# AlexanderGSC/gmres

Measured on AMD Instinct MI355X. Metric: Arnoldi iters/sec + HBM GB/s, 4096² Poisson-2D fp64, GMRES(m=95), higher is better.
Workload: dtype f64

## Files before the change

### gmres_amd/_native.py

```python
from __future__ import annotations

import ctypes
import os
import sys
import re

PKG = os.path.dirname(os.path.abspath(__file__))
LIB_DIR = os.environ.get("GK_LIB_DIR") or os.path.join(PKG, "lib")
HIP_SO = os.path.join(LIB_DIR, "libgmres_hip.so")
FHOST_SO = os.path.join(LIB_DIR, "libgmres_fhost.so")
HEADER = os.path.join(os.path.dirname(PKG), "include", "gmres_hip.h")

GK_OK = 0
GK_ERR_COMM = -6
GK_TUNE_PROJ_NT = 0
GK_TUNE_STENCIL_BLOCKS = 2
GK_TUNE_SR_BLOCKS = 28
GK_TUNE_SR_TWO_LEVEL = 29
GK_TUNE_XCHG_TIMEOUT_MS = 7
GK_TUNE_RES, GK_TUNE_RES_R2, GK_TUNE_RES_SHARE, GK_TUNE_RES_TIMEOUT_MS = 8, 9, 10, 11
GK_TUNE_VERR_ORDER = 14
GK_TUNE_HH_FUSE = 15
GK_TUNE_CHEB_STEN = 16
GK_TUNE_SPIN_WAIT = 18
GK_TUNE_GRAPH = 19
GK_TUNE_RES_QDEF = 20
GK_TUNE_RES_PC = 21
GK_TUNE_RES_FOLD = 22
GK_TUNE_RES_BLOCK = 23
GK_TUNE_WATCHDOG_MS = 24
GK_TUNE_HH_NORM_ORDER = 25
GK_TUNE_RES_PF = 27
GK_PREC_IDENTITY, GK_PREC_CBPR2, GK_PREC_CHEB = 0, 1, 2
(GK_KID_PROJ, GK_KID_STENCIL, GK_KID_SCALE, GK_KID_UPDATE, GK_KID_COMM, GK_KID_OTHER, GK_KID_RES, GK_KID_PREC,
 GK_KID_HALO, GK_KID_GRAPH) = range(10)
GK_KID_SR = 10
SR_PASS_NAMES = ["sr_cg_p", "sr_cg_x", "sr_cg_z", "sr_bi_p", "sr_bi_pc", "sr_bi_s", "sr_bi_sc", "sr_st1", "sr_st2",
                 "sr_bi_x", "sr_bi_pe", "sr_bi_se", "sr_dot", "sr_cg_xz", "sr_bi_pz", "sr_bi_sz"]
KID_NAMES = ["proj", "stencil", "scale", "update", "comm", "other", "res", "prec", "halo", "graph"] + SR_PASS_NAMES
GK_SR_PCG, GK_SR_BICGSTAB = 0, 1
COMM_KINDS = {0: None, 1: "rccl", 2: "local-group", 3: "xgmi-device-exchange"}
RES_VARIANTS = {0: None, 1: "prefetch", 2: "pairs", 3: "pairs+lds", 4: "w-only", 5: "w+column", 6: "blocked"}
RES_INFO_KEYS = ["variant", "G", "r2", "l2", "pf", "cw", "wo", "nt", "r2e", "l2e", "lds", "nres2", "unused12", "cheb_sten", "wt", "blk"]

c_int, c_double, c_ll, c_vp = ctypes.c_int, ctypes.c_double, ctypes.c_longlong, ctypes.c_void_p
_dp = ctypes.POINTER(ctypes.c_double)
_ip = ctypes.POINTER(ctypes.c_int)

_hip = None
_fhost = None


class GkError(RuntimeError):
    pass


def header_symbols() -> list[str]:
    txt = open(HEADER).read()
    return sorted(set(re.findall(r"^\s*(?:int|const char \*)\s*(gk_\w+)\s*\(", txt, re.M)))


_SIGS = {
    "gk_last_error": (ctypes.c_char_p, []),
    "gk_version": (c_int, []),
    "gk_runtime_info": (c_int, [_ip, _ip, _ip, ctypes.c_char_p, ctypes.c_char_p, c_int]),
    "gk_create": (c_int, [c_int, c_int, c_int, c_int, c_int, ctypes.POINTER(c_vp)]),
    "gk_destroy": (c_int, [c_vp]),
    "gk_comm_unique_id": (c_int, [ctypes.c_char_p]),
    "gk_comm_init": (c_int, [c_vp, c_int, c_int, c_int, ctypes.c_char_p]),
    "gk_local_size": (c_int, [c_vp, ctypes.POINTER(c_ll)]),
    "gk_comm_info": (c_int, [c_vp, _ip, _ip]),
    "gk_peer_info": (c_int, [c_int, c_int, _ip, _ip, _ip]),
    "gk_comm_latency": (c_int, [c_vp, c_int, _dp, _dp]),
    "gk_group_create": (c_int, [c_int, ctypes.POINTER(c_vp)]),
    "gk_group_destroy": (c_int, [c_vp]),
    "gk_comm_init_local": (c_int, [c_vp, c_vp, c_int, c_int]),
    "gk_comm_init_xgmi": (c_int, [c_vp, c_int, c_int, c_int]),
    "gk_xchg_handle": (c_int, [c_vp, ctypes.c_char_p]),
    "gk_xchg_open": (c_int, [c_vp, ctypes.c_char_p]),
    "gk_xchg_local": (c_int, [c_vp]),
    "gk_xchg_enable": (c_int, [c_vp, c_int]),
    "gk_xchg_selftest": (c_int, [c_vp, c_int]),
    "gk_set_precond": (c_int, [c_vp, c_int, _dp, c_int, c_int]),
    "gk_set_rhs": (c_int, [c_vp, _dp]),
    "gk_set_rhs_ones": (c_int, [c_vp]),
    "gk_rhs_norm": (c_int, [c_vp, _dp]),
    "gk_zero_x": (c_int, [c_vp]),
    "gk_get_x": (c_int, [c_vp, _dp]),
    "gk_get_basis": (c_int, [c_vp, c_int, c_int, _dp]),
    "gk_set_x": (c_int, [c_vp, _dp]),
    "gk_apply": (c_int, [c_vp, c_int, _dp, _dp]),
    "gk_true_residual": (c_int, [c_vp, _dp]),
    "gk_mgs_cycle_start": (c_int, [c_vp, _dp]),
    "gk_mgs_step": (c_int, [c_vp, c_int, _dp]),
    "gk_mgs_step_async": (c_int, [c_vp, c_int]),
    "gk_mgs_step_wait": (c_int, [c_vp, c_int, _dp]),
# ... 157 lines not shown
```

### gmres_amd/csrc/gk_api.hip

```cpp
#include <dlfcn.h>
#include <hip/hip_runtime.h>
#include <rccl/rccl.h>

#include <algorithm>
#include <atomic>
#include <chrono>
#include <cmath>
#include <condition_variable>
#include <cstdarg>
#include <cstdlib>
#include <mutex>
#include <cstdio>
#include <cstring>
#include <deque>
#include <string>
#include <vector>

#include "../../include/gmres_hip.h"
#include "gk_blk.hpp"
#include "gk_kernels.hpp"
#include "gk_sr.hpp"

using gk::i64;

// ... 54 lines not shown
    hipStream_t st = nullptr;
    double *V = nullptr;
    double *w = nullptr, *z = nullptr, *aux = nullptr, *dA = nullptr, *dB = nullptr;
    double *x = nullptr, *b = nullptr, *vj = nullptr, *hlo = nullptr, *hhi = nullptr;
    double *dh = nullptr;
    double *zline = nullptr;
    double *red = nullptr;
    double *hcol = nullptr;
    double *ydev = nullptr;
    double *hb = nullptr;
    double *scal = nullptr;
    double *hcol_host = nullptr;
    double *hall = nullptr;
    double *hallh = nullptr;
    double *hallh_dev = nullptr;
    std::vector<hipEvent_t> ev_step;
    double *Vb = nullptr;
    double *gram_slab = nullptr, *gram_out = nullptr;
    short2 *gram_pairs = nullptr;
    int gram_nblk = 0;
    int pkind = GK_PREC_IDENTITY, pdeg = 8;
    double p0 = 8.2, p1 = 0.2;
    int nranks = 1, rank = 0, max_lines = 0;
    int min_lines = 0;
    ncclComm_t comm = nullptr;
    bool comm_ok = false;
    gk_group *lg = nullptr;
    hipEvent_t lev_a = nullptr, lev_b = nullptr;
    double *lscratch = nullptr;
    gk::u64 *xs_buf = nullptr;
    i64 xs_words = 0;
    gk::XsPeers xs_peers{};
    std::vector<void *> xs_mapped;
    bool xs_ready = false, xs_on = false, xs_broken = false;
    unsigned xs_seq = 0, xs_hseq = 0;
    int *xs_err = nullptr, *xs_err_dev = nullptr;
    long long xs_tick_per_ms = 100000;
    int xs_timeout_ms = 20000;
    gk::u64 xs_timeout = 0;
    gk::u64 *res_gath = nullptr;
    double *res_gm = nullptr;
    int tune_res_blk = 1;
    int tune_res_pf = 0;
    int pend_res_blk = 0, pend_res_pf = -1;
    int watchdog_ms = 0;
    bool broken = false;
    unsigned *hold_word = nullptr, *hold_word_dev = nullptr;
    int *res_err = nullptr, *res_err_dev = nullptr;
    unsigned res_tag = 1;
    int res_cus = 0;
    int tune_res = -1;
    int tune_res_r2 = 0;
    int tune_res_lds = 1;
    int tune_res_wonly = -1;
    int tune_verr_order = 1;
    int tune_hh_fuse = 1;
    int tune_hh_norm_order = 0;
    int res_share = 1;
    int res_timeout_ms = 20000;
    bool res_broken = false;
    gk::u64 *res_stamps = nullptr;
    bool res_split = false;
    gk::u64 *res_trace = nullptr;
    int res_trace_j = 0, res_trace_mode = -1;
    int res_trace_g = 0, res_trace_np = 0;
    int vec = 2, JT = 16;
    dim3 sgrid;
    int sr_JT = 64, tune_sr_blocks = 0;
    int tune_sr_two = 1;
    bool sr_two = false;
    dim3 sr_sgrid;
    int np_sr = 0;
    int np_st = 0, np_pj = 0, nblk_stream = 0;
    int last_np = 0;
    int tune_cheb_fused = 1;
    int tune_cheb_sten = 1;
    int tune_spin_wait = 1;
    int tune_graph = 1;
    int tune_res_qdef = -1;
    int tune_res_pc = -1;
    int tune_res_fold = 1;
    std::vector<hipGraphExec_t> gstep;
    std::vector<unsigned> gxs;
    int gkey = -1;
    unsigned graph_seq0 = 0;
    unsigned *xs_seqdev = nullptr;
    bool capturing = false;
    int tune_nt = -1, tune_pj_blocks = 0, tune_st_blocks = 0;
    bool nt_auto = false;
    int tune_blocked = 0, tune_unr = 0;
    int prof_every = 1;
    bool prof_on_step = true;
    bool cycle_mgs = false, cycle_hh = false;
    double beta0 = -1.0;
    bool prof = false;
    std::vector<hipEvent_t> ev0, ev1;
    std::vector<int> evk;
    int nev = 0;
    double prof_ms[GK_NKID] = {0};
    long long prof_n[GK_NKID] = {0};
    gk::SrDev *sr_dev = nullptr;
    gk::SrMirror *sr_mir = nullptr, *sr_mir_dev = nullptr;
    double *sr_hist = nullptr;
    int sr_hist_len = 0;
    int sr_solver = -1, sr_par = 0, sr_queued = 0, sr_maxit = 0;
    std::deque<hipEvent_t> sr_pend;
// ... 440 lines not shown
    else
        launch_proj_u<NT, 4>(c, mode, w, va, vb, pin, npin, pout, hslot, coef, tail0, hstore);
}

int proj(gk_ctx *c, int mode, double *w, const double *va, const double *vb, const double *pin,
         int npin, double *pout, double *hslot, double coef, i64 tail0 = 0, int hstore = 0) {
    ProfScope ps(c, GK_KID_PROJ);
    if (c->tune_nt > 0 || (c->tune_nt < 0 && c->nt_auto))
        launch_proj<true>(c, mode, w, va, vb, pin, npin, pout, hslot, coef, tail0, hstore);
    else
        launch_proj<false>(c, mode, w, va, vb, pin, npin, pout, hslot, coef, tail0, hstore);
    LAUNCHCHK();
    return GK_OK;
}

int scale(gk_ctx *c, double *out, const double *w, const double *pin, int npin, double *hslot,
          double *hcopy = nullptr, const double *hsrc = nullptr, int ncopy = 0, bool pin_norm = false) {
    ProfScope ps(c, GK_KID_SCALE);
    gk::k_scale<<<c->nblk_stream, gk::TPB, 0, c->st>>>(out, w, pin, npin, hslot, c->nloc, hcopy, hsrc, ncopy,
                                                       pin_norm ? 1 : 0);
    LAUNCHCHK();
    return GK_OK;
}

int norm2_seq(gk_ctx *c, const double *x, i64 n, double *out) {
    ProfScope ps(c, GK_KID_OTHER);
    gk::k_norm2_seq<<<1, gk::TPB, 0, c->st>>>(x, n, out);
    LAUNCHCHK();
    return GK_OK;
}

int finalize(gk_ctx *c, const double *pin, int npin, double *out, int take_sqrt) {
    ProfScope ps(c, GK_KID_OTHER);
    gk::k_finalize<<<1, gk::TPB, 0, c->st>>>(pin, npin, out, take_sqrt);
    LAUNCHCHK();
    return GK_OK;
}

constexpr int RES_LDS_MIN = 96 * 1024;
constexpr int RES_L2 = 18;
constexpr int RES_R2_BIG = 12;

#ifndef GK_RES_RW
#define GK_RES_RW 89
#endif
#ifndef GK_RES_LW
#define GK_RES_LW 39
#endif
constexpr int RES_RW = GK_RES_RW, RES_LW = GK_RES_LW, RES_LW_HH = 38;
#ifndef GK_RES_RW_HH
#define GK_RES_RW_HH 90
#endif
constexpr int RES_RW_HH = GK_RES_RW_HH;

struct ResPlan {
    int G = 0, r2 = 0, l2 = 0;
    int r2e = 0, l2e = 0;
    bool pf = false, nt = false, cw = false, wo = false;
    bool pc = false;
    bool pcs = false;
    int blk = 0;
    int bvar = -1;
    int wt = 0;
    i64 nres2 = 0;
    int lds = 0;
};

#ifndef GK_RES_PC_NT
#define GK_RES_PC_NT 512
#endif
#ifndef GK_RES_PC_WB
#define GK_RES_PC_WB (GK_RES_PC_NT == 512 ? 4 : 8)
#endif
#ifndef GK_RES_PC_WB_HH
#define GK_RES_PC_WB_HH (GK_RES_PC_NT == 512 ? 4 : 6)
#endif
#ifndef GK_RES_PC_TOUCH
#define GK_RES_PC_TOUCH 0
#endif
#ifndef GK_RES_PC_RX
#define GK_RES_PC_RX (GK_RES_PC_NT == 512 ? 4 : 26)
#endif
constexpr int RES_PC_NT = GK_RES_PC_NT;
static_assert(RES_PC_NT == 256 || RES_PC_NT == 512, "column-cache workgroups of one or two waves per SIMD");
#ifndef GK_RES_PC_RX_MGS
#define GK_RES_PC_RX_MGS (GK_RES_PC_NT == 512 ? 6 : GK_RES_PC_RX)
#endif
constexpr int RES_PC_RW = RES_PC_NT == 512 ? 32 : 64, RES_PC_RX = GK_RES_PC_RX, RES_PC_LX = RES_PC_NT == 512 ? 19 : 38;
constexpr int RES_PC_RX_MGS = GK_RES_PC_RX_MGS;
constexpr int RES_PC_WB = GK_RES_PC_WB, RES_PC_WB_HH = GK_RES_PC_WB_HH, RES_PC_TOUCH = GK_RES_PC_TOUCH;
#ifndef GK_RES_PC_SMALL
#define GK_RES_PC_SMALL 1
#endif
constexpr bool RES_PCS = GK_RES_PC_SMALL != 0 && RES_PC_NT == 512;
constexpr int RES_PCS_RW = 16, RES_PCS_RX = 16, RES_PCS_LX = 0;

i64 pc_bytes(i64 n2, int G, bool hh) {
    if (RES_PCS && n2 <= (i64)G * RES_PCS_RW * RES_PC_NT) return 8 * n2;
    const int rx = hh ? RES_PC_RX : RES_PC_RX_MGS;
    const i64 cap = (i64)G * RES_PC_RW * RES_PC_NT, cached = (i64)G * (rx + RES_PC_LX) * RES_PC_NT;
    const i64 r = std::min(n2, cap), c = std::min(r, cached);
    return 8 * c + 16 * (r - c) + 32 * (n2 - r);
}

i64 pairs_bytes(i64 n2, int G) {
    const i64 rp = (i64)G * RES_R2_BIG * gk::RT, lp = (i64)G * RES_L2 * gk::RT;
    auto clamp = [](i64 v) { return v < 0 ? (i64)0 : v; };
    const i64 pr = std::min(n2, rp), pl = std::min(clamp(n2 - rp), lp), ps = clamp(n2 - rp - lp);
    return 8 * pr + 16 * pl + 32 * ps;
}

i64 wonly_bytes(i64 n2, int G) {
    const i64 rw = (i64)G * (RES_RW + RES_LW) * gk::WT;
    const i64 wr = std::min(n2, rw), ws = n2 > rw ? n2 - rw : 0;
    return 16 * wr + 32 * ws;
}

bool wonly_pays(i64 n2, int G) { return wonly_bytes(n2, G) < pairs_bytes(n2, G); }

void plan_resident(i64 nloc, int gmax, int cap, int tune_lds, int tune_wonly, bool hh, bool nt, ResPlan &p,
                   int tune_pc = -1, int tune_blk = 1, int tune_pf = 0) {
    const i64 n2 = nloc / 2;
    const i64 dcw = gk::RT - 64;
    const int gcw = (int)std::max<i64>(1, std::min<i64>(gmax, (n2 + 2 * dcw - 1) / (2 * dcw)));
    const i64 need = (n2 + (i64)gcw * dcw - 1) / ((i64)gcw * dcw);
    p = ResPlan{};
    static const int pfs[] = {2, 4, 8};
    for (int s : pfs)
        if (s <= cap && (p.r2 == 0 || p.r2 < need)) p.r2 = s;
    auto spread = [&](i64 dt, int rmax, int lmax) {
        const i64 nchf = n2 / dt, G = p.G;
        p.r2e = (int)std::min<i64>(rmax, (nchf + G - 1) / G);
        const i64 rest = std::max<i64>(0, nchf - G * p.r2e);
        p.l2e = (int)std::min<i64>(lmax, (rest + G - 1) / G);
        p.nres2 = std::min<i64>(nchf, G * (p.r2e + p.l2e)) * dt;
    };
    const int var = gk::blk_variant((n2 + (i64)gmax * 512 - 1) / ((i64)gmax * 512));
    const bool pf = !hh && tune_blk == 1 && var != gk::BLK_WONLY && tune_pf > 0;
    if (!hh && (tune_blk > 1 || pf)) {
        p.G = gmax;
        const gk::BlkGeom g = gk::blk_geom(var, tune_blk);
        p.blk = tune_blk;
        p.bvar = var;
        p.wt = g.nt;
        spread(g.nt, g.rw, g.lw);
        p.r2 = g.rx;
        p.l2 = g.lx;
        p.lds = (g.lw + tune_blk * (g.lx + g.pfx)) * g.nt * (int)sizeof(double2);
        p.nt = true;
        return;
    }
    const bool pc_fits = n2 <= (i64)gmax * RES_PC_RW * RES_PC_NT;
    const i64 other_bytes = std::min(pairs_bytes(n2, gmax), wonly_bytes(n2, gmax));
    const bool pc_pays = pc_fits && (RES_PC_NT == 512 ? pc_bytes(n2, gmax, hh) < other_bytes
                                                      : 3 * pc_bytes(n2, gmax, hh) <= 2 * other_bytes);
    if (p.r2 >= need || cap < RES_R2_BIG) {
        p.G = gcw;
        p.pf = p.cw = true;
        spread(dcw, p.r2, 0);
    } else if (tune_wonly <= 0 && (tune_pc > 0 ? pc_fits : (tune_pc < 0 && pc_pays))) {
        p.G = gmax;
        p.pc = true;
        p.wt = RES_PC_NT;
        spread(RES_PC_NT, RES_PC_RW, 0);
        p.pcs = RES_PCS && p.r2e <= RES_PCS_RW;
        p.r2 = p.pcs ? RES_PCS_RX : (hh ? RES_PC_RX : RES_PC_RX_MGS);
        p.l2 = p.pcs ? RES_PCS_LX : RES_PC_LX;
        p.lds = p.l2 * RES_PC_NT * (int)sizeof(double2);
        p.nt = true;
        return;
    } else if (tune_wonly > 0 || (tune_wonly < 0 && wonly_pays(n2, gmax))) {
        p.G = gmax;
        p.wo = true;
        p.wt = gk::WT;
        p.r2 = 0;
        spread(gk::WT, hh ? RES_RW_HH : RES_RW, hh ? RES_LW_HH : RES_LW);
        p.lds = (hh ? RES_LW_HH : RES_LW) * gk::WT * (int)sizeof(double2);
        p.nt = true;
        return;
    } else {
        p.G = gmax;
        p.r2 = RES_R2_BIG;
        const i64 dt = gk::RT, regs = (i64)p.G * RES_R2_BIG * dt;
        p.l2 = (tune_lds && n2 / dt * dt > regs) ? RES_L2 : 0;
        spread(dt, RES_R2_BIG, p.l2);
    }
    p.lds = std::max<int>(RES_LDS_MIN, p.l2 * (p.cw ? gk::RT - 64 : gk::RT) * (int)sizeof(double2));
    p.wt = gk::RT;
    p.nt = nt;
}

bool nt_auto_for(i64 max_nloc) { return max_nloc * 8 > (i64)48 * 1024 * 1024; }

bool res_plan(gk_ctx *c, ResPlan &p, bool hh = false) {
    if (c->tune_res == 0 || c->res_broken || c->m > gk::RHMAX || c->res_cus <= 0 || c->res_gath == nullptr)
        return false;
    if (collective(c) && !(c->xs_on && c->nranks > 1)) return false;
    if (c->tune_res < 0 && c->res_share > 1) return false;
    const int gmax = std::max(1, std::min(gk::RGMAX, c->res_cus / std::max(1, c->res_share)));
    const int cap = c->tune_res_r2 > 0 ? c->tune_res_r2 : RES_R2_BIG;
    plan_resident(c->nloc, gmax, cap, c->tune_res_lds, c->tune_res_wonly, hh,
                  c->tune_nt > 0 || (c->tune_nt < 0 && c->nt_auto), p, c->tune_res_pc, c->tune_res_blk, c->tune_res_pf);
    if (p.wo && !hh && c->m + 1 > gk::WO_HMAX) return false;
    return true;
}

enum { RPI_VARIANT = 0, RPI_G, RPI_R2, RPI_L2, RPI_PF, RPI_CW, RPI_WO, RPI_NT, RPI_R2E, RPI_L2E, RPI_LDS, RPI_NRES2, RPI_UNUSED12,
       RPI_CHEB_STEN, RPI_WT, RPI_BLK };
void plan_info(const ResPlan &p, bool on, long long *info) {
    for (int k = 0; k < GK_RES_INFO_LEN; ++k) info[k] = 0;
    if (!on) return;
    info[RPI_VARIANT] = p.bvar >= 0 ? GK_RES_BLOCKED
                        : p.pc    ? GK_RES_WCOL
                                  : (p.wo ? GK_RES_WONLY
                                          : (p.pf ? GK_RES_PREFETCH : (p.l2 > 0 ? GK_RES_PAIRS_LDS : GK_RES_PAIRS)));
    info[RPI_BLK] = p.bvar >= 0 ? p.blk : 1;
    info[RPI_G] = p.G;
    info[RPI_R2] = p.r2;
    info[RPI_L2] = p.l2;
    info[RPI_PF] = p.pf;
    info[RPI_CW] = p.cw;
    info[RPI_WO] = p.wo;
    info[RPI_NT] = p.nt;
    info[RPI_R2E] = p.r2e;
    info[RPI_L2E] = p.l2e;
    info[RPI_LDS] = p.lds;
    info[RPI_NRES2] = p.nres2;
    info[RPI_WT] = p.wt;
}

constexpr int ATTR_DEVS = 64;

template <int R2, int L2, bool PF, bool NT, bool CW, int MODE>
int launch_res_m(gk_ctx *c, const ResPlan &p, const gk::ResArgs &a) {
    static std::atomic<int> attr[ATTR_DEVS];
    if (c->dev < 0 || c->dev >= ATTR_DEVS) return set_err(GK_ERR_ARG, "device id %d out of range", c->dev);
    if (attr[c->dev].load() < p.lds) {
        HIPCHK(hipFuncSetAttribute(reinterpret_cast<const void *>(&gk::k_mgs_res<R2, L2, PF, NT, CW, MODE>),
                                   hipFuncAttributeMaxDynamicSharedMemorySize, p.lds));
        attr[c->dev] = p.lds;
    }
    gk::k_mgs_res<R2, L2, PF, NT, CW, MODE><<<p.G, gk::RT, p.lds, c->st>>>(a);
    LAUNCHCHK();
    return GK_OK;
}

template <int R2, int L2, bool PF, bool NT, bool CW>
int launch_res_t(gk_ctx *c, const ResPlan &p, const gk::ResArgs &a) {
    switch (a.mode) {
        case gk::RES_HH_UP: return launch_res_m<R2, L2, PF, NT, CW, gk::RES_HH_UP>(c, p, a);
        case gk::RES_HH_DOWN: return launch_res_m<R2, L2, PF, NT, CW, gk::RES_HH_DOWN>(c, p, a);
        default: return launch_res_m<R2, L2, PF, NT, CW, gk::RES_MGS>(c, p, a);
    }
}

template <int MODE>
int launch_wres_m(gk_ctx *c, const ResPlan &p, const gk::ResArgs &a) {
    constexpr int RW = MODE == gk::RES_MGS ? RES_RW : RES_RW_HH;
    constexpr int LW = MODE == gk::RES_MGS ? RES_LW : RES_LW_HH;
    constexpr int WBT = MODE == gk::RES_MGS ? gk::WB : gk::WB_HH;
    static std::atomic<int> attr[ATTR_DEVS];
    if (c->dev < 0 || c->dev >= ATTR_DEVS) return set_err(GK_ERR_ARG, "device id %d out of range", c->dev);
    if (attr[c->dev].load() < p.lds) {
        HIPCHK(hipFuncSetAttribute(reinterpret_cast<const void *>(&gk::k_mgs_wres<RW, LW, MODE, WBT>),
                                   hipFuncAttributeMaxDynamicSharedMemorySize, p.lds));
        attr[c->dev] = p.lds;
    }
    gk::k_mgs_wres<RW, LW, MODE, WBT><<<p.G, gk::WT, p.lds, c->st>>>(a);
    LAUNCHCHK();
    return GK_OK;
}

int launch_wres(gk_ctx *c, const ResPlan &p, const gk::ResArgs &a) {
    switch (a.mode) {
        case gk::RES_HH_UP: return launch_wres_m<gk::RES_HH_UP>(c, p, a);
        case gk::RES_HH_DOWN: return launch_wres_m<gk::RES_HH_DOWN>(c, p, a);
        default: return launch_wres_m<gk::RES_MGS>(c, p, a);
    }
}

template <int RW, int RX, int LX, int MODE>
int launch_wpc_k(gk_ctx *c, const ResPlan &p, const gk::ResArgs &a) {
    constexpr int WBT = MODE == gk::RES_MGS ? RES_PC_WB : RES_PC_WB_HH;
    static std::atomic<int> attr[ATTR_DEVS];
    if (c->dev < 0 || c->dev >= ATTR_DEVS) return set_err(GK_ERR_ARG, "device id %d out of range", c->dev);
    if (p.r2e > RW || p.lds < LX * RES_PC_NT * (int)sizeof(double2))
        return set_err(GK_ERR_STATE, "column-cache plan (%d chunks, %d B LDS) does not fit k_mgs_wpc<%d,%d,%d>", p.r2e,
                       p.lds, RW, RX, LX);
    if (p.lds > 0 && attr[c->dev].load() < p.lds) {
        HIPCHK(hipFuncSetAttribute(
            reinterpret_cast<const void *>(&gk::k_mgs_wpc<RW, RX, LX, MODE, WBT, RES_PC_TOUCH, RES_PC_NT>),
            hipFuncAttributeMaxDynamicSharedMemorySize, p.lds));
        attr[c->dev] = p.lds;
    }
    gk::k_mgs_wpc<RW, RX, LX, MODE, WBT, RES_PC_TOUCH, RES_PC_NT><<<p.G, RES_PC_NT, p.lds, c->st>>>(a);
    LAUNCHCHK();
    return GK_OK;
}

template <int MODE>
int launch_wpc_m(gk_ctx *c, const ResPlan &p, const gk::ResArgs &a) {
    if constexpr (RES_PCS) {
        if (p.pcs) return launch_wpc_k<RES_PCS_RW, RES_PCS_RX, RES_PCS_LX, MODE>(c, p, a);
    }
    return launch_wpc_k<RES_PC_RW, MODE == gk::RES_MGS ? RES_PC_RX_MGS : RES_PC_RX, RES_PC_LX, MODE>(c, p, a);
}

int launch_res(gk_ctx *c, const ResPlan &p, const gk::ResArgs &a) {
    if (p.bvar >= 0) {
        if (a.mode != gk::RES_MGS) return set_err(GK_ERR_STATE, "the blocked step is the MGS-R step's only");
        const int e = gk::blk_launch(p.bvar, p.blk, a, p.G, p.lds, c->dev, c->st);
        if (e != 0)
            return set_err(GK_ERR_HIP, "k_mgs_blk (S=%d, variant %d): %s", p.blk, p.bvar,
                           hipGetErrorString(static_cast<hipError_t>(e)));
        return GK_OK;
    }
    if (p.wo) return launch_wres(c, p, a);
    if (p.pc) {
        switch (a.mode) {
            case gk::RES_HH_UP: return launch_wpc_m<gk::RES_HH_UP>(c, p, a);
            case gk::RES_HH_DOWN: return launch_wpc_m<gk::RES_HH_DOWN>(c, p, a);
            default: return launch_wpc_m<gk::RES_MGS>(c, p, a);
        }
    }
#define GK_RES_CASE(R, L, PFV, CWV)                                                                 \
    if (p.r2 == R && p.l2 == L && p.pf == PFV && p.cw == CWV)                                      \
        return p.nt ? launch_res_t<R, L, PFV, true, CWV>(c, p, a) : launch_res_t<R, L, PFV, false, CWV>(c, p, a);
    GK_RES_CASE(2, 0, true, true)
    GK_RES_CASE(4, 0, true, true)
    GK_RES_CASE(8, 0, true, true)
// ... 1413 lines not shown
    return GK_OK;
}

int gk_apply(gk_ctx *c, int what, const double *in, double *out) {
    CHK(check_ctx(c));
    if (in == nullptr || out == nullptr || (what != 0 && what != 1)) return set_err(GK_ERR_ARG, "bad gk_apply args");
    HIPCHK(hipSetDevice(c->dev));
    c->cycle_mgs = c->cycle_hh = false;
    if (what == 0) {
        HIPCHK(hipMemcpyAsync(c->vj, in, sizeof(double) * c->nloc, hipMemcpyHostToDevice, c->st));
        CHK(halo(c, c->vj));
        gk::StArgs a{};
        a.x = c->vj;
        a.y = c->w;
        CHK(stencil(c, gk::OP_PLAIN, gk::ACC_NONE, a));
    } else {
        HIPCHK(hipMemcpyAsync(c->z, in, sizeof(double) * c->nloc, hipMemcpyHostToDevice, c->st));
        if (c->pkind == GK_PREC_IDENTITY) {
            HIPCHK(hipMemcpyAsync(c->w, c->z, sizeof(double) * c->nloc, hipMemcpyDeviceToDevice, c->st));
        } else {
            CHK(precond_sweeps(c, c->w, gk::ACC_NONE, nullptr, nullptr));
        }
    }
    HIPCHK(hipMemcpyAsync(out, c->w, sizeof(double) * c->nloc, hipMemcpyDeviceToHost, c->st));
    CHK(sync_st(c));
    if (c->prof) CHK(prof_harvest(c));
    return GK_OK;
}

int gk_set_tuning(gk_ctx *c, int key, int value) {
    CHK(check_ctx(c));
    switch (key) {
        case GK_TUNE_PROJ_NT: c->tune_nt = value < 0 ? -1 : (value != 0); break;
        case GK_TUNE_PROJ_BLOCKS: c->tune_pj_blocks = value; break;
        case GK_TUNE_STENCIL_BLOCKS: c->tune_st_blocks = value; break;
        case GK_TUNE_CHEB_FUSED: c->tune_cheb_fused = value != 0; break;
        case GK_TUNE_PROJ_BLOCKED: c->tune_blocked = value != 0; break;
        case GK_TUNE_XCHG_TIMEOUT_MS:
            if (value < 1) return set_err(GK_ERR_ARG, "timeout must be >= 1 ms");
            xs_set_timeout(c, value);
            break;
        case GK_TUNE_RES: c->tune_res = value < 0 ? -1 : (value != 0); break;
        case GK_TUNE_RES_R2:
            if (value != 0 && value != 2 && value != 4 && value != 8 && value != 12)
                return set_err(GK_ERR_ARG, "resident cap must be 0 (auto), 2, 4, 8 or 12");
            c->tune_res_r2 = value;
            break;
        case GK_TUNE_RES_SHARE:
            if (value < 1) return set_err(GK_ERR_ARG, "share must be >= 1");
            c->res_share = value;
            break;
        case GK_TUNE_RES_LDS: c->tune_res_lds = value != 0; break;
        case GK_TUNE_RES_WONLY: c->tune_res_wonly = value < 0 ? -1 : (value != 0); break;
        case GK_TUNE_HH_FUSE: c->tune_hh_fuse = value != 0; break;
        case GK_TUNE_CHEB_STEN: c->tune_cheb_sten = value != 0; break;
        case GK_TUNE_SPIN_WAIT: c->tune_spin_wait = value != 0; break;
        case GK_TUNE_GRAPH: c->tune_graph = value != 0; break;
        case GK_TUNE_RES_QDEF: c->tune_res_qdef = value < 0 ? -1 : (value != 0); break;
        case GK_TUNE_RES_PC: c->tune_res_pc = value < 0 ? -1 : (value != 0); break;
        case GK_TUNE_RES_FOLD: c->tune_res_fold = value != 0; break;
        case GK_TUNE_WATCHDOG_MS: c->watchdog_ms = std::max(0, value); break;
        case GK_TUNE_HH_NORM_ORDER: c->tune_hh_norm_order = value != 0; break;
        case GK_TUNE_RES_BLOCK:
            if (value != 1 && value != 2 && value != 4)
                return set_err(GK_ERR_ARG, "GK_TUNE_RES_BLOCK %d: blocks of 1 (strict MGS-R), 2 or 4 projections", value);
            if (c->cycle_mgs)
                c->pend_res_blk = value;
            else
                c->tune_res_blk = value;
            break;
        case GK_TUNE_SR_BLOCKS: c->tune_sr_blocks = std::max(0, value); break;
        case GK_TUNE_SR_TWO_LEVEL: c->tune_sr_two = value != 0; break;
        case GK_TUNE_RES_PF:
            if (c->cycle_mgs)
                c->pend_res_pf = value != 0;
            else
                c->tune_res_pf = value != 0;
            break;
        case GK_TUNE_VERR_ORDER: c->tune_verr_order = value != 0; break;
        case GK_TUNE_RES_TIMEOUT_MS:
            if (value < 1) return set_err(GK_ERR_ARG, "timeout must be >= 1 ms");
            c->res_timeout_ms = value;
            break;
        case GK_TUNE_PROJ_UNROLL:
            if (value != 0 && value != 2 && value != 4 && value != 8)
                return set_err(GK_ERR_ARG, "unroll must be 0 (auto), 2, 4 or 8");
            c->tune_unr = value;
            break;
        default: return set_err(GK_ERR_ARG, "unknown tuning key %d", key);
    }
    set_geometry(c);
    graph_reset(c);
    return GK_OK;
}


int gk_profile_enable(gk_ctx *c, int enable) {
    CHK(check_ctx(c));
    if (!enable) CHK(prof_harvest(c));
    c->prof = enable != 0;
    c->prof_every = enable > 1 ? enable : 1;
    c->prof_on_step = true;
    return GK_OK;
}

int gk_profile_reset(gk_ctx *c) {
// ... 852 lines not shown
```

### gmres_amd/csrc/gk_kernels.hpp

```cpp
#pragma once
#include "gk_common.hpp"
#include "gk_cheb.hpp"
#include "gk_res.hpp"

namespace gk {

enum { PJ_DOT = 0, PJ_AXPY = 1, PJ_AXPY_DOT = 2, PJ_AXPY_NORM = 3 };


template <int MODE, bool NT = false, int U = UNR>
__global__ __launch_bounds__(TPB) void k_proj(double *__restrict__ w, const double *__restrict__ va,
                                              const double *__restrict__ vb,
                                              const double *__restrict__ pin, int npin,
                                              double *__restrict__ pout, double *__restrict__ hslot,
                                              double coef, i64 n, i64 tail0, int blocked,
                                              int hstore) {
    __shared__ double sm[WAVES];
    const i64 n2 = n >> 1;
    double2 *__restrict__ W2 = reinterpret_cast<double2 *>(w);
    const double2 *__restrict__ A2 = reinterpret_cast<const double2 *>(va);
    const double2 *__restrict__ B2 = reinterpret_cast<const double2 *>(vb);
    i64 lo, hi, step;
    if (blocked) {
        const i64 chunk = (i64)TPB * U;
// ... 876 lines not shown
        return;
    }
    const double hn = sqrt(h);
    double2 *__restrict__ O2 = reinterpret_cast<double2 *>(a.vout);
    if (data) {
#pragma unroll
        for (int k = 0; k < R2; ++k)
            if (c0 + k < cend)
                O2[(c0 + k) * DT + td] = hn != 0.0 ? double2{wr[k].x / hn, wr[k].y / hn} : double2{0.0, 0.0};
        if constexpr (L2 > 0) {
            for (int k = 0; k < L2; ++k)
                if (l0 + k < lend) {
                    const double2 v = lw[k * DT + td];
                    O2[(l0 + k) * DT + td] = hn != 0.0 ? double2{v.x / hn, v.y / hn} : double2{0.0, 0.0};
                }
        }
        for (i64 e = sbase; e < n2; e += sstride) {
            const double2 v = W2[e];
            O2[e] = hn != 0.0 ? double2{v.x / hn, v.y / hn} : double2{0.0, 0.0};
        }
        if ((a.n & 1) && blockIdx.x == gridDim.x - 1 && td == 0) a.vout[a.n - 1] = hn != 0.0 ? a.w[a.n - 1] / hn : 0.0;
    }
    clk.finish(a.stamps, mode);
    if (blockIdx.x == 0) {
        __syncthreads();
        for (int k = t; k < j; k += RT) {
            a.hs[k] = hsh[k];
            a.hcopy[k] = hsh[k];
        }
        if (t == 0) {
            a.hs[j] = hn;
            a.hcopy[j] = hn;
        }
    }
}

constexpr int WT = 256;
#ifndef GK_RES_WB
#define GK_RES_WB 8
#endif
constexpr int WB = GK_RES_WB;
#ifndef GK_RES_WB_HH
#define GK_RES_WB_HH 6
#endif
constexpr int WB_HH = GK_RES_WB_HH;
#ifndef GK_RES_TOUCH
#define GK_RES_TOUCH 24
#endif
constexpr int TOUCH = GK_RES_TOUCH;
#ifndef GK_RES_TOUCH_MGS
#define GK_RES_TOUCH_MGS 28
#endif
constexpr int TOUCH_MGS = GK_RES_TOUCH_MGS;
#ifndef GK_RES_QNT
#define GK_RES_QNT 0
#endif
constexpr bool RES_QNT = GK_RES_QNT != 0;
#ifndef GK_RES_TOUCH_PACE
#define GK_RES_TOUCH_PACE 24
#endif
constexpr int TOUCH_PACE = GK_RES_TOUCH_PACE;
#ifndef GK_RES_TOUCH_PACE_HH
#define GK_RES_TOUCH_PACE_HH 0
#endif
constexpr int TOUCH_PACE_HH = GK_RES_TOUCH_PACE_HH;

template <int RW, int LW, int MODE, int WBT = WB>
__global__ __launch_bounds__(WT, 1) void k_mgs_wres(ResArgs a) {
    extern __shared__ double2 lw[];
    __shared__ double sm[WT / 64];
    __shared__ double bc[1];
    __shared__ int okf;
    __shared__ int xdone;
    __shared__ double hsh[MODE == RES_MGS ? WO_HMAX : 1];
    const int t = threadIdx.x;
    constexpr int mode = MODE;
    constexpr int PACE = MODE == RES_MGS ? TOUCH_PACE : TOUCH_PACE_HH;
    constexpr int TCH = MODE == RES_MGS ? TOUCH_MGS : TOUCH;
    const int j = a.j, np = res_np(mode, j);
    const i64 n2 = a.n >> 1, ld2 = a.ld >> 1;
    const i64 nch = a.nres2 / WT;
    const i64 bq = blockIdx.x;
    const i64 c0 = bq * a.r2e, cend = c0 + a.r2e < nch ? c0 + a.r2e : nch;
    const i64 l0 = (i64)gridDim.x * a.r2e + bq * a.l2e, lend = l0 + a.l2e < nch ? l0 + a.l2e : nch;
    const i64 tail0 = mode == RES_HH_UP ? a.tail0 : 0;
    const double2 *__restrict__ V2 = reinterpret_cast<const double2 *>(a.V);
    double2 *__restrict__ W2 = reinterpret_cast<double2 *>(a.w);
    ResClock clk;
    clk.start(a.stamps);
    int touch_sink = 0;
    const i64 sstride = (i64)gridDim.x * WT;
    const i64 sbase = a.nres2 + (i64)res_stream_wg() * WT + t;
    double2 wr[RW];
    if (mode == RES_HH_DOWN && a.unit_init) {
        const i64 u = a.unit_e;
        auto unit2 = [&](i64 e2) { return double2{2 * e2 == u ? 1.0 : 0.0, 2 * e2 + 1 == u ? 1.0 : 0.0}; };
#pragma unroll
        for (int k = 0; k < RW; ++k) wr[k] = (c0 + k < cend) ? unit2((c0 + k) * WT + t) : double2{0.0, 0.0};
        for (int k = 0; k < LW; ++k)
            if (l0 + k < lend) lw[k * WT + t] = unit2((l0 + k) * WT + t);
        for (i64 e = sbase; e < n2; e += sstride) W2[e] = unit2(e);
        if ((a.n & 1) && blockIdx.x == gridDim.x - 1 && t == 0) a.w[a.n - 1] = (a.n - 1 == u) ? 1.0 : 0.0;
    } else {
#pragma unroll
        for (int k = 0; k < RW; ++k) wr[k] = (c0 + k < cend) ? W2[(c0 + k) * WT + t] : double2{0.0, 0.0};
        for (int k = 0; k < LW; ++k)
            if (l0 + k < lend) lw[k * WT + t] = W2[(l0 + k) * WT + t];
    }
    auto red = [&](double &acc, const double2 &v, const double2 &b, int kind, i64 e2, bool chk) {
        if (kind == RK_DOT) {
            acc = acc + v.x * b.x;
            acc = acc + v.y * b.y;
        } else if (kind == RK_NORM) {
            sq_acc(acc, v, e2, tail0, chk);
        }
    };
    auto pass = [&](double ch, int i, int q, int kind) -> double {
        const double2 *__restrict__ A2 = V2 + (i64)i * ld2;
        const double2 *__restrict__ B2 = V2 + (i64)q * ld2;
        const bool dot = kind == RK_DOT;
        double acc = 0.0;
        auto rbatch = [&](const int k0) {
            double2 av[WBT], bv[WBT];
#pragma unroll
            for (int u = 0; u < WBT; ++u) {
                const i64 c = c0 + k0 + u;
                if (k0 + u < RW && c < cend) {
                    av[u] = ldv<true>(A2 + c * WT + t);
                    if (dot) bv[u] = ldv<RES_QNT>(B2 + c * WT + t);
                }
            }
#pragma unroll
            for (int u = 0; u < WBT; ++u) {
                const int k = k0 + u;
                if (k < RW && c0 + k < cend) {
                    wr[k].x = wr[k].x - ch * av[u].x;
                    wr[k].y = wr[k].y - ch * av[u].y;
                    red(acc, wr[k], bv[u], kind, (c0 + k) * WT + t, mode == RES_HH_UP && c0 + k == 0);
                }
            }
        };
        auto lbatch = [&](const int k0, const int kend) {
            double2 av[WBT], bv[WBT];
#pragma unroll
            for (int u = 0; u < WBT; ++u) {
                const i64 c = l0 + k0 + u;
                if (k0 + u < kend && c < lend) {
                    av[u] = ldv<true>(A2 + c * WT + t);
                    if (dot) bv[u] = ldv<RES_QNT>(B2 + c * WT + t);
                }
            }
#pragma unroll
            for (int u = 0; u < WBT; ++u) {
                const int k = k0 + u;
                if (k < kend && l0 + k < lend) {
                    double2 wv = lw[k * WT + t];
                    wv.x = wv.x - ch * av[u].x;
                    wv.y = wv.y - ch * av[u].y;
                    lw[k * WT + t] = wv;
                    red(acc, wv, bv[u], kind, (l0 + k) * WT + t, mode == RES_HH_UP && l0 + k == 0);
                }
            }
        };
#pragma unroll
        for (int k0 = 0; k0 < RW; k0 += WBT) rbatch(k0);
        for (int k0 = 0; k0 < LW; k0 += WBT) lbatch(k0, LW);
        for (i64 e0 = sbase; e0 < n2; e0 += 2 * sstride) {
            double2 wv[2], av[2], bv[2];
#pragma unroll
            for (int u = 0; u < 2; ++u) {
                const i64 e = e0 + u * sstride;
                if (e < n2) {
                    wv[u] = W2[e];
                    av[u] = ldv<true>(A2 + e);
// ... 116 lines not shown
            return;
        }
        const double s = sqrt(h);
        const i64 f = tail0;
        auto fix1 = [&](double &x, i64 g) {
            if (g < f) {
                a.hb[g] = x;
                x = 0.0;
            } else if (g == f) {
                a.hb[g] = x;
                const double dl = (x > 0.0) ? s : -s;
                x = x + dl;
            }
        };
        auto fix_sq = [&](double &acc2, double2 &v, i64 e2, bool chk) {
            if (chk) {
                fix1(v.x, 2 * e2);
                fix1(v.y, 2 * e2 + 1);
            }
            acc2 = acc2 + v.x * v.x;
            acc2 = acc2 + v.y * v.y;
        };
        const i64 cfix = f >= 0 ? f / (2 * WT) : -1;
        double acc2 = 0.0;
#pragma unroll
        for (int k = 0; k < RW; ++k)
            if (c0 + k < cend) fix_sq(acc2, wr[k], (c0 + k) * WT + t, c0 + k <= cfix);
        for (int k = 0; k < LW; ++k)
            if (l0 + k < lend) {
                double2 v = lw[k * WT + t];
                const bool chk = l0 + k <= cfix;
                fix_sq(acc2, v, (l0 + k) * WT + t, chk);
                if (chk) lw[k * WT + t] = v;
            }
        for (i64 e = sbase; e < n2; e += sstride) {
            double2 v = W2[e];
            const bool chk = 2 * e <= f;
            fix_sq(acc2, v, e, chk);
            if (chk) W2[e] = v;
        }
        if ((a.n & 1) && blockIdx.x == gridDim.x - 1 && t == 0) {
            double x = a.w[a.n - 1];
            if (a.n - 1 <= f) {
                fix1(x, a.n - 1);
                a.w[a.n - 1] = x;
            }
            acc2 = acc2 + x * x;
        }
        ok = reduce(acc2, h, -1);
        if (!ok) return;
    }
    const double hn = sqrt(h);
    double2 *__restrict__ O2 = reinterpret_cast<double2 *>(a.vout);
#pragma unroll
    for (int k = 0; k < RW; ++k)
        if (c0 + k < cend)
            O2[(c0 + k) * WT + t] = hn != 0.0 ? double2{wr[k].x / hn, wr[k].y / hn} : double2{0.0, 0.0};
    for (int k = 0; k < LW; ++k)
        if (l0 + k < lend) {
            const double2 v = lw[k * WT + t];
            O2[(l0 + k) * WT + t] = hn != 0.0 ? double2{v.x / hn, v.y / hn} : double2{0.0, 0.0};
        }
    for (i64 e = sbase; e < n2; e += sstride) {
        const double2 v = W2[e];
        O2[e] = hn != 0.0 ? double2{v.x / hn, v.y / hn} : double2{0.0, 0.0};
    }
    if ((a.n & 1) && blockIdx.x == gridDim.x - 1 && t == 0) a.vout[a.n - 1] = hn != 0.0 ? a.w[a.n - 1] / hn : 0.0;
    clk.finish(a.stamps, mode);
    if (mode == RES_MGS && blockIdx.x == 0) {
        __syncthreads();
        for (int k = t; k < j; k += WT) {
            a.hs[k] = hsh[k];
            a.hcopy[k] = hsh[k];
        }
        if (t == 0) {
            a.hs[j] = hn;
            a.hcopy[j] = hn;
        }
    }
}


template <int RW, int RX, int LX, int MODE, int WBT = 8, int TCHP = 0, int NT = WT>
__global__ __launch_bounds__(NT, 1) void k_mgs_wpc(ResArgs a) {
    static_assert(RX <= RW && RX + LX <= RW, "the column cache covers register chunks of w only");
    extern __shared__ double2 lx[];
    __shared__ int xdone;
    __shared__ double sm[NT / 64];
    __shared__ double bc[1];
    __shared__ int okf;
    __shared__ double hsh[RHMAX + 1];
    const int t = threadIdx.x;
    constexpr int mode = MODE;
    const int j = a.j, np = res_np(mode, j);
    const i64 n2 = a.n >> 1, ld2 = a.ld >> 1;
    const i64 nch = a.nres2 / NT;
    const i64 c0 = (i64)blockIdx.x * a.r2e, cend = c0 + a.r2e < nch ? c0 + a.r2e : nch;
    const i64 tail0 = mode == RES_HH_UP ? a.tail0 : 0;
    const double2 *__restrict__ V2 = reinterpret_cast<const double2 *>(a.V);
    double2 *__restrict__ W2 = reinterpret_cast<double2 *>(a.w);
    ResClock clk;
    clk.start(a.stamps);
    const i64 sstride = (i64)gridDim.x * NT;
    const i64 sbase = a.nres2 + (i64)res_stream_wg() * NT + t;
    double2 wr[RW], xc[RX > 0 ? RX : 1];
    {
        const double2 *__restrict__ C2 = V2 + (i64)res_col(mode, j, 0) * ld2;
#pragma unroll
        for (int k = 0; k < RW; ++k) wr[k] = (c0 + k < cend) ? W2[(c0 + k) * NT + t] : double2{0.0, 0.0};
#pragma unroll
        for (int k = 0; k < RX; ++k) xc[k] = (c0 + k < cend) ? ldv<true>(C2 + (c0 + k) * NT + t) : double2{0.0, 0.0};
        for (int k = 0; k < LX; ++k)
// ... 178 lines not shown
```

### include/gmres_hip.h

```cpp
#ifndef GMRES_HIP_H
#define GMRES_HIP_H

#ifdef __cplusplus
extern "C" {
#endif

#define GK_OK 0
#define GK_ERR_ARG (-1)
#define GK_ERR_HIP (-2)
#define GK_ERR_RCCL (-3)
#define GK_ERR_STATE (-4)
#define GK_ERR_NOMEM (-5)
#define GK_ERR_COMM (-6)

#define GK_PREC_IDENTITY 0
#define GK_PREC_CBPR2 1
#define GK_PREC_CHEB 2

#define GK_KID_PROJ 0
#define GK_KID_STENCIL 1
#define GK_KID_SCALE 2
#define GK_KID_UPDATE 3
#define GK_KID_COMM 4
#define GK_KID_OTHER 5
// ... 77 lines not shown
int gk_sr_start(gk_ctx *ctx, int solver, double tol, int max_iter);
int gk_sr_iterate(gk_ctx *ctx, int k);
int gk_sr_status(gk_ctx *ctx, int wait, int *executed, int *done, double *res);
int gk_sr_history(gk_ctx *ctx, double *hist, int n);

int gk_profile_enable(gk_ctx *ctx, int enable);
int gk_profile_reset(gk_ctx *ctx);
int gk_profile_read(gk_ctx *ctx, int kid, double *total_ms, long long *launches);
int gk_profile_res_split(gk_ctx *ctx, int mode, int which, double *pass_ms, double *wait_ms, double *total_ms,
                         long long *launches);
int gk_profile_res_wg(gk_ctx *ctx, int which, double *pass_ms, double *wait_ms, int maxwg, int *nwg);
int gk_profile_res_trace(gk_ctx *ctx, int arm, int j, int mode, unsigned long long *out, int maxwg, int maxx,
                         int *nwg, int *nx, double *tick_per_ms);
int gk_sync(gk_ctx *ctx);

#define GK_RES_NONE 0
#define GK_RES_PREFETCH 1
#define GK_RES_PAIRS 2
#define GK_RES_PAIRS_LDS 3
#define GK_RES_WONLY 4
#define GK_RES_WCOL 5
#define GK_RES_BLOCKED 6
#define GK_RES_INFO_LEN 16
int gk_res_plan_query(long long nloc, int cus, int share, int hh, int nt, int block, long long *info);
int gk_res_info(gk_ctx *ctx, int hh, long long *info);

#define GK_TUNE_PROJ_NT 0
#define GK_TUNE_PROJ_BLOCKS 1
#define GK_TUNE_STENCIL_BLOCKS 2
#define GK_TUNE_PROJ_BLOCKED 4
#define GK_TUNE_PROJ_UNROLL 5
#define GK_TUNE_CHEB_FUSED 6
#define GK_TUNE_XCHG_TIMEOUT_MS 7
#define GK_TUNE_RES 8
#define GK_TUNE_RES_R2 9
#define GK_TUNE_RES_SHARE 10
#define GK_TUNE_RES_TIMEOUT_MS 11
#define GK_TUNE_RES_LDS 12
#define GK_TUNE_RES_WONLY 13
#define GK_TUNE_VERR_ORDER 14
#define GK_TUNE_HH_FUSE 15
#define GK_TUNE_CHEB_STEN 16
#define GK_TUNE_SPIN_WAIT 18
#define GK_TUNE_GRAPH 19
#define GK_TUNE_RES_QDEF 20
#define GK_TUNE_RES_PC 21
#define GK_TUNE_RES_FOLD 22
#define GK_TUNE_RES_BLOCK 23
#define GK_TUNE_WATCHDOG_MS 24
#define GK_TUNE_HH_NORM_ORDER 25
#define GK_TUNE_RES_PF 27
#define GK_TUNE_SR_BLOCKS 28
#define GK_TUNE_SR_TWO_LEVEL 29
int gk_set_tuning(gk_ctx *ctx, int key, int value);
int gk_debug_hold_stream(gk_ctx *ctx, int hold);

int gk_poisson5(int nside, int nlines, const double *x, const double *halo_lo,
                const double *halo_hi, double *y, void *stream);
int gk_precond_apply(int nside, int kind, const double *params, int degree, const double *r,
                     double *z, double *scratch, void *stream);
int gk_mgs_project(long long n, double *w, const double *va, double *result, void *stream);
int gk_dot(long long n, const double *a, const double *b, double *result, void *stream);

#ifdef __cplusplus
}
#endif
#endif
```

Baseline: 250.1.

## Add software-pipelined MGS pass in resident w-only kernel with explicit vmcnt waits

Adds a pipelined variant of the resident w-only MGS projection pass. Loads of V_i and V_q chunks are issued D ahead with inline global_load_dwordx4 and gated by explicit s_waitcnt vmcnt counts, so memory latency overlaps with the update and reduction. It is enabled by default only when the plan exactly fills all register and LDS chunks, and bounds checks are dropped on that path. Hand-written asm waitcnt accounting and compiler-barrier tricks add correctness risk and register pressure.

```diff
diff --git a/gmres_amd/_native.py b/gmres_amd/_native.py
--- a/gmres_amd/_native.py
+++ b/gmres_amd/_native.py
@@ -31,6 +31,7 @@
 GK_TUNE_WATCHDOG_MS = 24
 GK_TUNE_HH_NORM_ORDER = 25
 GK_TUNE_RES_PF = 27
+GK_TUNE_RES_PIPE = 30
 GK_PREC_IDENTITY, GK_PREC_CBPR2, GK_PREC_CHEB = 0, 1, 2
 (GK_KID_PROJ, GK_KID_STENCIL, GK_KID_SCALE, GK_KID_UPDATE, GK_KID_COMM, GK_KID_OTHER, GK_KID_RES, GK_KID_PREC,
  GK_KID_HALO, GK_KID_GRAPH) = range(10)
@@ -41,7 +42,7 @@
 GK_SR_PCG, GK_SR_BICGSTAB = 0, 1
 COMM_KINDS = {0: None, 1: "rccl", 2: "local-group", 3: "xgmi-device-exchange"}
 RES_VARIANTS = {0: None, 1: "prefetch", 2: "pairs", 3: "pairs+lds", 4: "w-only", 5: "w+column", 6: "blocked"}
-RES_INFO_KEYS = ["variant", "G", "r2", "l2", "pf", "cw", "wo", "nt", "r2e", "l2e", "lds", "nres2", "unused12", "cheb_sten", "wt", "blk"]
+RES_INFO_KEYS = ["variant", "G", "r2", "l2", "pf", "cw", "wo", "nt", "r2e", "l2e", "lds", "nres2", "pipe", "cheb_sten", "wt", "blk"]
 
 c_int, c_double, c_ll, c_vp = ctypes.c_int, ctypes.c_double, ctypes.c_longlong, ctypes.c_void_p
 _dp = ctypes.POINTER(ctypes.c_double)
diff --git a/gmres_amd/csrc/gk_api.hip b/gmres_amd/csrc/gk_api.hip
--- a/gmres_amd/csrc/gk_api.hip
+++ b/gmres_amd/csrc/gk_api.hip
@@ -130,6 +130,7 @@
     int tune_res = -1;
     int tune_res_r2 = 0;
     int tune_res_lds = 1;
+    int tune_res_pipe = -1;
     int tune_res_wonly = -1;
     int tune_verr_order = 1;
     int tune_hh_fuse = 1;
@@ -676,6 +677,11 @@
 #define GK_RES_RW_HH 90
 #endif
 constexpr int RES_RW_HH = GK_RES_RW_HH;
+#ifndef GK_RES_PIPE
+#define GK_RES_PIPE 1
+#endif
+constexpr bool RES_PIPE = GK_RES_PIPE != 0;
+constexpr bool RES_PIPE_OK = 2 * (gk::PIPE_D - 1) <= 63 && RES_RW + RES_LW > gk::PIPE_D && !gk::RES_QNT;
 
 struct ResPlan {
     int G = 0, r2 = 0, l2 = 0;
@@ -686,6 +692,7 @@
     int blk = 0;
     int bvar = -1;
     int wt = 0;
+    bool pipe = false;
     i64 nres2 = 0;
     int lds = 0;
 };
@@ -743,7 +750,7 @@
 bool wonly_pays(i64 n2, int G) { return wonly_bytes(n2, G) < pairs_bytes(n2, G); }
 
 void plan_resident(i64 nloc, int gmax, int cap, int tune_lds, int tune_wonly, bool hh, bool nt, ResPlan &p,
-                   int tune_pc = -1, int tune_blk = 1, int tune_pf = 0) {
+                   int tune_pc = -1, int tune_blk = 1, int tune_pf = 0, int tune_pipe = -1) {
     const i64 n2 = nloc / 2;
     const i64 dcw = gk::RT - 64;
     const int gcw = (int)std::max<i64>(1, std::min<i64>(gmax, (n2 + 2 * dcw - 1) / (2 * dcw)));
@@ -801,6 +808,8 @@
         spread(gk::WT, hh ? RES_RW_HH : RES_RW, hh ? RES_LW_HH : RES_LW);
         p.lds = (hh ? RES_LW_HH : RES_LW) * gk::WT * (int)sizeof(double2);
         p.nt = true;
+        p.pipe = RES_PIPE_OK && !hh && (tune_pipe < 0 ? RES_PIPE : tune_pipe != 0) && p.r2e == RES_RW &&
+                 p.l2e == RES_LW && nloc % 2 == 0 && n2 == (i64)p.G * (RES_RW + RES_LW) * gk::WT && p.nres2 == n2;
         return;
     } else {
         p.G = gmax;
@@ -824,12 +833,13 @@
     const int gmax = std::max(1, std::min(gk::RGMAX, c->res_cus / std::max(1, c->res_share)));
     const int cap = c->tune_res_r2 > 0 ? c->tune_res_r2 : RES_R2_BIG;
     plan_resident(c->nloc, gmax, cap, c->tune_res_lds, c->tune_res_wonly, hh,
-                  c->tune_nt > 0 || (c->tune_nt < 0 && c->nt_auto), p, c->tune_res_pc, c->tune_res_blk, c->tune_res_pf);
+                  c->tune_nt > 0 || (c->tune_nt < 0 && c->nt_auto), p, c->tune_res_pc, c->tune_res_blk, c->tune_res_pf,
+                  c->tune_res_pipe);
     if (p.wo && !hh && c->m + 1 > gk::WO_HMAX) return false;
     return true;
 }
 
-enum { RPI_VARIANT = 0, RPI_G, RPI_R2, RPI_L2, RPI_PF, RPI_CW, RPI_WO, RPI_NT, RPI_R2E, RPI_L2E, RPI_LDS, RPI_NRES2, RPI_UNUSED12,
+enum { RPI_VARIANT = 0, RPI_G, RPI_R2, RPI_L2, RPI_PF, RPI_CW, RPI_WO, RPI_NT, RPI_R2E, RPI_L2E, RPI_LDS, RPI_NRES2, RPI_PIPE,
        RPI_CHEB_STEN, RPI_WT, RPI_BLK };
 void plan_info(const ResPlan &p, bool on, long long *info) {
     for (int k = 0; k < GK_RES_INFO_LEN; ++k) info[k] = 0;
@@ -851,6 +861,7 @@
     info[RPI_LDS] = p.lds;
     info[RPI_NRES2] = p.nres2;
     info[RPI_WT] = p.wt;
+    info[RPI_PIPE] = p.pipe;
 }
 
 constexpr int ATTR_DEVS = 64;
@@ -878,19 +889,19 @@
     }
 }
 
-template <int MODE>
+template <int MODE, bool PIPE = false>
 int launch_wres_m(gk_ctx *c, const ResPlan &p, const gk::ResArgs &a) {
     constexpr int RW = MODE == gk::RES_MGS ? RES_RW : RES_RW_HH;
     constexpr int LW = MODE == gk::RES_MGS ? RES_LW : RES_LW_HH;
-    constexpr int WBT = MODE == gk::RES_MGS ? gk::WB : gk::WB_HH;
+    constexpr int WBT = PIPE ? gk::PIPE_D : (MODE == gk::RES_MGS ? gk::WB : gk::WB_HH);
     static std::atomic<int> attr[ATTR_DEVS];
     if (c->dev < 0 || c->dev >= ATTR_DEVS) return set_err(GK_ERR_ARG, "device id %d out of range", c->dev);
     if (attr[c->dev].load() < p.lds) {
-        HIPCHK(hipFuncSetAttribute(reinterpret_cast<const void *>(&gk::k_mgs_wres<RW, LW, MODE, WBT>),
+        HIPCHK(hipFuncSetAttribute(reinterpret_cast<const void *>(&gk::k_mgs_wres<RW, LW, MODE, WBT, PIPE>),
                                    hipFuncAttributeMaxDynamicSharedMemorySize, p.lds));
         attr[c->dev] = p.lds;
     }
-    gk::k_mgs_wres<RW, LW, MODE, WBT><<<p.G, gk::WT, p.lds, c->st>>>(a);
+    gk::k_mgs_wres<RW, LW, MODE, WBT, PIPE><<<p.G, gk::WT, p.lds, c->st>>>(a);
     LAUNCHCHK();
     return GK_OK;
 }
@@ -899,7 +910,16 @@
     switch (a.mode) {
         case gk::RES_HH_UP: return launch_wres_m<gk::RES_HH_UP>(c, p, a);
         case gk::RES_HH_DOWN: return launch_wres_m<gk::RES_HH_DOWN>(c, p, a);
-        default: return launch_wres_m<gk::RES_MGS>(c, p, a);
+        default:
+            if constexpr (RES_PIPE_OK) {
+                if (p.pipe) {
+                    if (p.r2e != RES_RW || p.l2e != RES_LW || (a.n & 1) || a.nres2 != a.n / 2)
+                        return set_err(GK_ERR_STATE, "pipelined w-only step on a plan that is not full (%d + %d chunks)",
+                                       p.r2e, p.l2e);
+                    return launch_wres_m<gk::RES_MGS, true>(c, p, a);
+                }
+            }
+            return launch_wres_m<gk::RES_MGS>(c, p, a);
     }
 }
 
@@ -2419,6 +2439,7 @@
             break;
         case GK_TUNE_RES_LDS: c->tune_res_lds = value != 0; break;
         case GK_TUNE_RES_WONLY: c->tune_res_wonly = value < 0 ? -1 : (value != 0); break;
+        case GK_TUNE_RES_PIPE: c->tune_res_pipe = value < 0 ? -1 : (value != 0); break;
         case GK_TUNE_HH_FUSE: c->tune_hh_fuse = value != 0; break;
         case GK_TUNE_CHEB_STEN: c->tune_cheb_sten = value != 0; break;
         case GK_TUNE_SPIN_WAIT: c->tune_spin_wait = value != 0; break;
diff --git a/gmres_amd/csrc/gk_kernels.hpp b/gmres_amd/csrc/gk_kernels.hpp
--- a/gmres_amd/csrc/gk_kernels.hpp
+++ b/gmres_amd/csrc/gk_kernels.hpp
@@ -952,6 +952,10 @@
 #define GK_RES_TOUCH_MGS 28
 #endif
 constexpr int TOUCH_MGS = GK_RES_TOUCH_MGS;
+#ifndef GK_RES_TOUCH_MGS_PIPE
+#define GK_RES_TOUCH_MGS_PIPE 20
+#endif
+constexpr int TOUCH_MGS_PIPE = GK_RES_TOUCH_MGS_PIPE;
 #ifndef GK_RES_QNT
 #define GK_RES_QNT 0
 #endif
@@ -964,8 +968,21 @@
 #define GK_RES_TOUCH_PACE_HH 0
 #endif
 constexpr int TOUCH_PACE_HH = GK_RES_TOUCH_PACE_HH;
-
-template <int RW, int LW, int MODE, int WBT = WB>
+#ifndef GK_RES_PIPE_D
+#define GK_RES_PIPE_D 8
+#endif
+constexpr int PIPE_D = GK_RES_PIPE_D;
+
+template <class F, int... I>
+__device__ __forceinline__ void seq_apply(F &&f, std::integer_sequence<int, I...>) {
+    (f(std::integral_constant<int, I>{}), ...);
+}
+template <int N, class F>
+__device__ __forceinline__ void seq_for(F &&f) {
+    seq_apply(f, std::make_integer_sequence<int, N>{});
+}
+
+template <int RW, int LW, int MODE, int WBT = WB, bool PIPE = false>
 __global__ __launch_bounds__(WT, 1) void k_mgs_wres(ResArgs a) {
     extern __shared__ double2 lw[];
     __shared__ double sm[WT / 64];
@@ -976,7 +993,7 @@
     const int t = threadIdx.x;
     constexpr int mode = MODE;
     constexpr int PACE = MODE == RES_MGS ? TOUCH_PACE : TOUCH_PACE_HH;
-    constexpr int TCH = MODE == RES_MGS ? TOUCH_MGS : TOUCH;
+    constexpr int TCH = MODE == RES_MGS ? (PIPE ? TOUCH_MGS_PIPE : TOUCH_MGS) : TOUCH;
     const int j = a.j, np = res_np(mode, j);
     const i64 n2 = a.n >> 1, ld2 = a.ld >> 1;
     const i64 nch = a.nres2 / WT;
@@ -1003,9 +1020,9 @@
         if ((a.n & 1) && blockIdx.x == gridDim.x - 1 && t == 0) a.w[a.n - 1] = (a.n - 1 == u) ? 1.0 : 0.0;
     } else {
 #pragma unroll
-        for (int k = 0; k < RW; ++k) wr[k] = (c0 + k < cend) ? W2[(c0 + k) * WT + t] : double2{0.0, 0.0};
+        for (int k = 0; k < RW; ++k) wr[k] = (PIPE || c0 + k < cend) ? W2[(c0 + k) * WT + t] : double2{0.0, 0.0};
         for (int k = 0; k < LW; ++k)
-            if (l0 + k < lend) lw[k * WT + t] = W2[(l0 + k) * WT + t];
+            if (PIPE || l0 + k < lend) lw[k * WT + t] = W2[(l0 + k) * WT + t];
     }
     auto red = [&](double &acc, const double2 &v, const double2 &b, int kind, i64 e2, bool chk) {
         if (kind == RK_DOT) {
@@ -1015,11 +1032,70 @@
             sq_acc(acc, v, e2, tail0, chk);
         }
     };
+    const i64 wc0 = c0, wl0 = l0;
     auto pass = [&](double ch, int i, int q, int kind) -> double {
         const double2 *__restrict__ A2 = V2 + (i64)i * ld2;
         const double2 *__restrict__ B2 = V2 + (i64)q * ld2;
         const bool dot = kind == RK_DOT;
         double acc = 0.0;
+        i64 c0 = wc0, l0 = wl0;
+        if constexpr (PIPE) {
+            int zero = 0;
+            asm volatile("" : "+s"(zero));
+            c0 += zero;
+            l0 += zero;
+        }
+        if constexpr (PIPE) {
+            constexpr int D = WBT, NCH = RW + LW;
+            static_assert(MODE == RES_MGS && NCH > D && 2 * (D - 1) <= 63 && !RES_QNT,
+                          "pipelined pass: the MGS step, counts within vmcnt's 6 bits, V_q default policy");
+            d2v pa[D], pb[D];
+            const unsigned lo = (unsigned)t * (unsigned)sizeof(double2);
+            const double2 *Ar = A2 + c0 * WT, *Al = A2 + l0 * WT, *Br = B2 + c0 * WT, *Bl = B2 + l0 * WT;
+            __builtin_amdgcn_s_waitcnt(0x0f70);
+            auto held = [&](int k) { return k < RW ? c0 + k < cend : l0 + (k - RW) < lend; };
+            auto issue = [&](auto kc) {
+                constexpr int k = decltype(kc)::value;
+                const double2 *ap = k < RW ? Ar + k * WT : Al + (k - RW) * WT;
+                const double2 *bq = k < RW ? Br + k * WT : Bl + (k - RW) * WT;
+                const double2 *bp = dot ? bq : Ar;
+                d2v &da = pa[k % D], &db = pb[k % D];
+                const unsigned off = lo;
+                asm volatile("global_load_dwordx4 %0, %1, %2 nt" : "=v"(da) : "v"(off), "s"(ap));
+                asm volatile("global_load_dwordx4 %0, %1, %2" : "=v"(db) : "v"(off), "s"(bp));
+            };
+            auto wait = [&](auto kc) {
+                constexpr int k = decltype(kc)::value;
+                constexpr int younger = NCH - 1 - k < D - 1 ? NCH - 1 - k : D - 1;
+                d2v &da = pa[k % D], &db = pb[k % D];
+                asm volatile("s_waitcnt vmcnt(%2)" : "+v"(da), "+v"(db) : "i"(2 * younger));
+            };
+            auto consume = [&](auto kc) {
+                constexpr int k = decltype(kc)::value;
+                const double2 av{pa[k % D].x, pa[k % D].y}, bv{pb[k % D].x, pb[k % D].y};
+                if (!held(k)) return;
+                if constexpr (k < RW) {
+                    wr[k].x = wr[k].x - ch * av.x;
+                    wr[k].y = wr[k].y - ch * av.y;
+                    red(acc, wr[k], bv, kind, (c0 + k) * WT + t, false);
+                } else {
+                    constexpr int kl = k - RW;
+                    double2 wv = lw[kl * WT + t];
+                    wv.x = wv.x - ch * av.x;
+                    wv.y = wv.y - ch * av.y;
+                    lw[kl * WT + t] = wv;
+                    red(acc, wv, bv, kind, (l0 + kl) * WT + t, false);
+                }
+            };
+            seq_for<D>(issue);
+            seq_for<NCH>([&](auto kc) {
+                constexpr int k = decltype(kc)::value;
+                wait(kc);
+                consume(kc);
+                if constexpr (k + D < NCH) issue(std::integral_constant<int, k + D>{});
+            });
+            return acc;
+        }
         auto rbatch = [&](const int k0) {
             double2 av[WBT], bv[WBT];
 #pragma unroll
@@ -1242,12 +1318,17 @@
     }
     const double hn = sqrt(h);
     double2 *__restrict__ O2 = reinterpret_cast<double2 *>(a.vout);
+    if constexpr (PIPE) {
+        int zero = 0;
+        asm volatile("" : "+s"(zero));
+        O2 += zero;
+    }
 #pragma unroll
     for (int k = 0; k < RW; ++k)
-        if (c0 + k < cend)
+        if (PIPE || c0 + k < cend)
             O2[(c0 + k) * WT + t] = hn != 0.0 ? double2{wr[k].x / hn, wr[k].y / hn} : double2{0.0, 0.0};
     for (int k = 0; k < LW; ++k)
-        if (l0 + k < lend) {
+        if (PIPE || l0 + k < lend) {
             const double2 v = lw[k * WT + t];
             O2[(l0 + k) * WT + t] = hn != 0.0 ? double2{v.x / hn, v.y / hn} : double2{0.0, 0.0};
         }
diff --git a/include/gmres_hip.h b/include/gmres_hip.h
--- a/include/gmres_hip.h
+++ b/include/gmres_hip.h
@@ -153,6 +153,7 @@
 #define GK_TUNE_RES_PF 27
 #define GK_TUNE_SR_BLOCKS 28
 #define GK_TUNE_SR_TWO_LEVEL 29
+#define GK_TUNE_RES_PIPE 30
 int gk_set_tuning(gk_ctx *ctx, int key, int value);
 int gk_debug_hold_stream(gk_ctx *ctx, int hold);
 
```

Measured after the change: 261.1, median of 6. +4.4%, better.
